# yosungho/LineTR

Measured on AMD Instinct MI355X. Metric: line_descriptors_per_sec, higher is better.
Workload: dtype f32 in/out; GEMMs as 6 bf16-split MFMA products, fp32 accumulate (fp32-faithful); 1 GPU; cfg3: 64 pairs/GPU of 640x480, 200 lines/image -> 199 sub-lines x 21 tokens, d_model=256, seeded weights; pairs_per_gpu=64, collective=none

## Files before the change

### linetr_amd/csrc/linetr_net.hip

```cpp
#include <algorithm>
#include <array>
#include <numeric>
#include <set>

#include "lt_handle.h"
#include "lt_gemm.h"
#include "lt_gemm_split.h"
#include "lt_gemm_split16.h"
#include "lt_st_image.h"
#include "lt_gemm_small.h"
#include "lt_model.h"
#include "lt_attn.h"
#include "lt_attn_fused.h"
#include "lt_gemm_ws.h"
#include "lt_tokmlp.h"
#include "lt_token.h"
#include "lt_bntrain.h"

using namespace lt;

namespace {

const char* gemm_class_name(int precision, int tile, const GemmArgs& g, int groups) {
  static const auto names = [] {
// ... 197 lines not shown
  }
  return 0;
}

int nhwc_map(LinetrHandle* h, hipStream_t st, const float* dense_desc, int dense_is_nhwc, int n_images, int P, float* buf,
             const float*& nhwc) {
  nhwc = dense_desc;
  if (dense_is_nhwc) return LINETR_OK;
  ProfScope ps(h, st, "nchw_to_nhwc", 0, 2.0 * n_images * P * D * 4);
  hipLaunchKernelGGL(nchw_to_nhwc_kernel, dim3(cdiv(P, 64), D / 64, n_images), dim3(256), 0, st, dense_desc, buf, D, P);
  LT_LAUNCH_CHECK();
  nhwc = buf;
  return LINETR_OK;
}

struct TokenFront {
  const LinetrLineRec* recs; int K, N; double td; int T;
  const float *dense_desc, *dense_score;
  int n_images, height, width, align_corners, dense_is_nhwc;
  double clip_x, clip_y;
  float *sublines, *resp, *angle_sub;
  int* s2l_g;
  float* nhwc_buf;
  bool map_always;
  double tokenize_bytes;
  float *cpnt = nullptr, *cscore = nullptr; int n_pad_images = 0; int64_t first_pad = 0;
};
int token_front(LinetrHandle* h, hipStream_t st, const TokenFront& a, const LinetrTokens& out, const K2sTable& k2s, int32_t* d_sub2line,
                const float*& nhwc) {
  {
    ProfScope ps(h, st, "line_fill", 0, (double)a.K * 80 + (double)a.N * 8);
    hipLaunchKernelGGL(line_fill_kernel, dim3(cdiv(a.K, 256)), dim3(256), 0, st, a.recs, a.K, a.clip_x, a.clip_y, out.klines, out.length,
                       out.angles, a.s2l_g, d_sub2line);
    LT_LAUNCH_CHECK();
  }
  {
    ProfScope ps(h, st, "tokenize", 0, a.tokenize_bytes);
    hipLaunchKernelGGL(tokenize_kernel, dim3(a.N + cdiv(a.n_pad_images, 64) + (out.mat ? a.K : 0)), dim3(64), 0, st, a.recs, a.s2l_g, a.N,
                       a.td, a.T, a.height, a.width, a.clip_x, a.clip_y, a.dense_score, a.sublines, out.pnt, out.mask, a.resp, a.angle_sub,
                       out.score, a.cpnt, a.cscore, a.n_pad_images, a.first_pad, out.mat, k2s);
    LT_LAUNCH_CHECK();
  }
  const int Hc = a.height / 8, Wc = a.width / 8;
  nhwc = nullptr;
  if (a.map_always || out.desc)
    if (int e = nhwc_map(h, st, a.dense_desc, a.dense_is_nhwc, a.n_images, Hc * Wc, a.nhwc_buf, nhwc)) return e;
  if (out.desc) {
    const int64_t ntok = (int64_t)a.N * a.T;
    ProfScope ps(h, st, "sample_desc", 0, (double)ntok * D * 4 * 2);
    hipLaunchKernelGGL(sample_desc_kernel, dim3((unsigned)((ntok + 3) / 4)), dim3(256), 0, st, out.pnt, a.s2l_g, a.recs, ntok, a.T, nhwc,
                       Hc, Wc, a.align_corners, out.desc);
    LT_LAUNCH_CHECK();
  }
  return LINETR_OK;
}
}

extern "C" int64_t linetr_tokenize_workspace_bytes(int32_t n_images, int32_t height, int32_t width, int32_t N) {
  const int64_t P = (int64_t)(height / 8) * (width / 8);
  return align_up(n_images * P * D * 4, 256) + align_up((int64_t)std::max(N, 1) * 4, 256) + 256;
}

extern "C" int linetr_tokenize(LinetrHandle* h, const LinetrLineRec* d_recs, int32_t K, int32_t N, double td,
                               int32_t T, const float* d_dense_desc, const float* d_dense_score, int32_t n_images,
                               int32_t height, int32_t width, int32_t clip_height, int32_t clip_width, int32_t align_corners,
// ... 8 lines not shown
  if (T < 1 || T > 4096 || height % 8 || width % 8) return fail(LINETR_E_ARG, "tokenize: bad max_tokens / image size");
  if (out.mat && n_images != 1) return fail(LINETR_E_ARG, "tokenize: mat_klines2sublines of several images: use linetr_describe (it has the sub-line prefix sums)");
  K2sTable k2s;
  if (int e = k2s_table(out, n_images, K, N, nullptr, k2s, "tokenize")) return e;
  if (ws_bytes < linetr_tokenize_workspace_bytes(n_images, height, width, N))
    return fail(LINETR_E_WORKSPACE, "tokenize: workspace too small");
  hipStream_t st = (hipStream_t)stream;
  if (h) LT_HIP(hipSetDevice(h->device));
  const int64_t P = (int64_t)(height / 8) * (width / 8);
  TokenFront f{d_recs, K, N, td, T, d_dense_desc, d_dense_score, n_images, height, width, align_corners, dense_is_nhwc,
               (double)clip_width - 0.6, (double)clip_height - 0.6, out.sublines, out.resp, out.angle_sub};
  f.nhwc_buf = (float*)d_ws;
  f.s2l_g = (int*)((char*)d_ws + align_up(n_images * P * D * 4, 256));
  f.map_always = false;
  f.tokenize_bytes = (double)N * T * 16;
  const float* nhwc;
  return token_front(h, st, f, out, k2s, d_sub2line, nhwc);
}

extern "C" int64_t linetr_sample_descriptors_workspace_bytes(int32_t Hc, int32_t Wc, int32_t dense_is_nhwc) {
  return dense_is_nhwc ? 0 : align_up((int64_t)Hc * Wc * D * 4, 256);
}

extern "C" int linetr_sample_descriptors(LinetrHandle* h, const float* d_points, int64_t n, const float* d_dense_desc, int32_t Hc,
                                         int32_t Wc, int32_t align_corners, int32_t dense_is_nhwc, float* d_out, void* d_ws,
                                         int64_t ws_bytes, void* stream) {
  if (n < 0 || Hc <= 0 || Wc <= 0) return fail(LINETR_E_ARG, "sample_descriptors: bad shape");
  if (n == 0) return LINETR_OK;
  if (!d_points || !d_dense_desc || !d_out) return fail(LINETR_E_ARG, "sample_descriptors: null pointer");
  if (ws_bytes < linetr_sample_descriptors_workspace_bytes(Hc, Wc, dense_is_nhwc) || (!dense_is_nhwc && !d_ws))
    return fail(LINETR_E_WORKSPACE, "sample_descriptors: workspace too small");
  hipStream_t st = (hipStream_t)stream;
// ... 84 lines not shown
  hipStream_t stream[LinetrHandle::PIPE_STREAMS];
  hipEvent_t ev[LinetrHandle::PIPE_STREAMS - 1];
  int cut[LinetrHandle::PIPE_STREAMS - 1];
  int n_cuts = 0, next = 0;
};
int pipe_boundary(PipeStages* p, int pos, hipStream_t& st) {
  if (!p || p->next >= p->n_cuts || p->cut[p->next] != pos) return LINETR_OK;
  LT_HIP(hipEventRecord(p->ev[p->next], st));
  LT_HIP(hipStreamWaitEvent(p->stream[p->next + 1], p->ev[p->next], 0));
  st = p->stream[++p->next];
  return LINETR_OK;
}

struct TokenStage {
  const float *pnt = nullptr, *score = nullptr, *desc = nullptr;
  const float *cpnt = nullptr, *cscore = nullptr, *nhwc = nullptr;
  const LinetrLineRec* recs = nullptr;
  const int* sub2line_g = nullptr;
  int64_t rows = 0;
  int64_t first_pad = 0;
  int Hc = 0, Wc = 0, align_corners = 0;
  const BnTrain* bn = nullptr;
  PipeStages* pipe = nullptr;
};

bool fused_mlp_enabled(const LinetrModelConfig& c) { return c.enc_channels[1] == 64 && c.enc_channels[2] == 128; }

int mlp123_rows_per_wave(int64_t rows) {
  const int64_t waves = 256 * 4;
  return (int)std::max<int64_t>(cdiv((int)cdiv((int)rows, (int)waves), 32) * 32, 32);
}
// ... 122 lines not shown
  if (ts.bn) {
    int64_t off = 0;
    if ((e = pos_encoder_bn(h, st, word, *ts.bn, off))) return e;
    if ((e = pos_encoder_bn(h, st, line, *ts.bn, off))) return e;
  } else if (plan.both >= 0) {
    ProfScope ps(h, st, "pos_mlp_dual_bf16x6", 2.0 * rows * (3 * e0 + e0 * e1 + e1 * e2 + e2 * e3) + 2.0 * N * (5 * e0 + e0 * e1 + e1 * e2 + e2 * e3),
                 (double)rows * (12 + 4 * e3) + (double)N * (28 + 4 * e3));
    if ((e = tok_mlp_launch_dual(tok_mlp_args(h, word), tok_mlp_args(h, line), st))) return e;
  } else {
    if ((e = pos_encoder(h, st, word, plan.word))) return e;
    if ((e = pos_encoder(h, st, line, plan.line))) return e;
  }
  return run_gemm(h, st, h->lW5, N, {w.act[ENC_LINE][3], e3}, {w.lpos, D}, ACT_NONE);
}

enum { POOLK_DENSE = 0, POOLK_ONLINE = 1, POOLK_ONLINE_REV = 2, POOLK_SPLIT4 = 3 };
int cls_pool_plan(bool online, int N) { return !online ? POOLK_DENSE : N <= 2048 ? POOLK_SPLIT4 : POOLK_ONLINE_REV; }

int cls_pool_launch(LinetrHandle* h, hipStream_t st, int kernel, const TokenStage& ts, int n_images, int N, int T, const float* a4,
                    float* pooled) {
  const int64_t rows = ts.rows;
  if (kernel != POOLK_DENSE) {
    const double tap_bytes = std::min((double)n_images * ts.Hc * ts.Wc * D * 4, (double)rows * D * 4 * 4);
    ProfScope ps(h, st, "cls_pool_online", 2.0 * rows * (2.0 * HEADS * D * 2), tap_bytes + (double)rows * D * 4 + (double)N * HEADS * POOLW * 4);
    if (kernel == POOLK_SPLIT4)
      hipLaunchKernelGGL(cls_pool_online_kernel<4>, dim3(N), dim3(256), 0, st, ts.recs, ts.sub2line_g, ts.cpnt,
                         a4, ts.first_pad, N, T, ts.nhwc, ts.Hc, ts.Wc, ts.align_corners, h->pool, pooled, 0);
    else
      hipLaunchKernelGGL(cls_pool_online_kernel<1>, dim3(cdiv(N, 4)), dim3(256), 0, st, ts.recs, ts.sub2line_g, ts.cpnt,
                         a4, ts.first_pad, N, T, ts.nhwc, ts.Hc, ts.Wc, ts.align_corners, h->pool, pooled, kernel == POOLK_ONLINE_REV ? 1 : 0);
    LT_LAUNCH_CHECK();
  } else {
    ProfScope ps(h, st, "cls_pool", 2.0 * rows * (2.0 * HEADS * D * 2), (double)rows * D * 8);
    hipLaunchKernelGGL(cls_pool_kernel, dim3(N), dim3(256), HEADS * (T + 1) * sizeof(float), st, ts.desc, a4, T, h->pool, pooled);
    LT_LAUNCH_CHECK();
  }
  return LINETR_OK;
}

int cls_pooling(LinetrHandle* h, hipStream_t& st, const TokenStage& ts, int n_images, int N, int T, FwdWs& w) {
  if (int e = cls_pool_launch(h, st, cls_pool_plan(ts.cpnt != nullptr, N), ts, n_images, N, T, w.act[ENC_WORD][3], w.pooled)) return e;
  const GemmGroups heads{HEADS, DH, POOLW, DH};
  return run_gemm(h, st, h->Watt, N, {w.pooled, HEADS * POOLW}, {w.att, D}, ACT_NONE, nullptr, &heads);
}

int sentence(LinetrHandle* h, hipStream_t& st, int N, FwdWs& w) {
  const LinetrModelConfig& c = h->cfg;
  int e;
  {
    NormSpec ns; ns.mode = 1; ns.gamma = h->ln1g; ns.beta = h->ln1b; ns.eps = 1e-6f;
    if ((e = run_gemm_norm(h, st, h->Wfc, N, {w.att, D}, nullptr, w.fc, w.o, ns))) return e;
  }
  if ((e = run_gemm(h, st, h->Wf1, N, {w.o, D}, {w.f1, c.d_inner}, ACT_GELU))) return e;
  NormSpec ns; ns.mode = 1; ns.gamma = h->ln2g; ns.beta = h->ln2b; ns.add2 = w.lpos; ns.eps = 1e-6f;
  return run_gemm_norm(h, st, h->Wf2, N, {w.f1, c.d_inner}, w.o, w.f2, w.zA, ns);
}
// ... 178 lines not shown
  if (!d_bn_running) return fail(LINETR_E_ARG, "forward_train: null running statistics");
  if (!(momentum >= 0.f && momentum <= 1.f)) return fail(LINETR_E_ARG, "forward_train: momentum out of [0, 1]");
  BnTrain bt;
  bt.running = d_bn_running; bt.batch = d_bn_batch; bt.momentum = momentum;
  return forward_dense(h, "forward_train", *tok, h_cu, d_cu, n_images, T, d_line_desc, d_ws, ws_bytes, (hipStream_t)stream, &bt);
}


namespace {
struct DescWs { float *nhwc, *cpnt, *cscore, *sublines, *resp, *angle_sub; int* s2l_g; int64_t fwd_off, total; };
DescWs desc_layout(int n_images, int height, int width, int N, int64_t rows, char* base) {
  DescWs d;
  int64_t off = 0;
  auto take = [&](int64_t bytes) { char* p = base + off; off += align_up(bytes, 256); return p; };
  const int64_t P = (int64_t)(height / 8) * (width / 8);
  d.nhwc = (float*)take(n_images * P * D * 4);
  d.cpnt = (float*)take(rows * 8);
  d.cscore = (float*)take(rows * 4);
  d.sublines = (float*)take((int64_t)N * 16);
  d.resp = (float*)take((int64_t)N * 4);
  d.angle_sub = (float*)take((int64_t)N * 8);
  d.s2l_g = (int*)take((int64_t)N * 4);
  d.fwd_off = off;
  d.total = off;
  return d;
}
}

extern "C" int64_t linetr_describe_workspace_bytes(const LinetrHandle* h, int32_t n_images, int32_t height, int32_t width,
                                                   int32_t N, int64_t n_real) {
  if (!h) return -1;
// ... 22 lines not shown
  if (ws_bytes < linetr_describe_workspace_bytes(h, n_images, height, width, N, n_real))
    return fail(LINETR_E_WORKSPACE, "describe: workspace too small");
  const int64_t rows = n_real + n_images;
  if (rows > INT32_MAX / 8) return fail(LINETR_E_ARG, "describe: batch too large");
  LT_HIP(hipSetDevice(h->device));
  DescWs dw = desc_layout(n_images, height, width, N, rows, (char*)d_ws);
  FwdWs w = fwd_layout(h, N, rows, n_images, (char*)d_ws + dw.fwd_off);
  const int* cu_dev;
  if (int e = cu_on_device(h_cu, d_cu, n_images, w, st, cu_dev)) return e;
  TokenFront f{d_recs, K, N, td, T, d_dense_desc, d_dense_score, n_images, height, width, align_corners, dense_is_nhwc,
               (double)width - 0.6, (double)height - 0.6, out.sublines ? out.sublines : dw.sublines, out.resp ? out.resp : dw.resp,
               out.angle_sub ? out.angle_sub : dw.angle_sub};
  f.s2l_g = dw.s2l_g; f.nhwc_buf = dw.nhwc;
  f.map_always = true;
  f.tokenize_bytes = (double)n_real * 16;
  f.cpnt = dw.cpnt; f.cscore = dw.cscore; f.n_pad_images = n_images; f.first_pad = n_real;
  const float* nhwc_map;
  if (int e = token_front(h, st, f, out, k2s, d_sub2line, nhwc_map)) return e;
  TokenStage ts;
  ts.cpnt = dw.cpnt; ts.cscore = dw.cscore; ts.nhwc = nhwc_map; ts.recs = d_recs; ts.sub2line_g = dw.s2l_g;
  ts.rows = rows; ts.first_pad = n_real; ts.Hc = height / 8; ts.Wc = width / 8; ts.align_corners = align_corners;
  ts.pipe = pipe;
  if (int e = pipe_boundary(pipe, CUT_TOKENS, st)) return e;
  return forward_core(h, st, ts, f.sublines, f.resp, f.angle_sub, h_cu, cu_dev, n_images, N, T, d_line_desc, w);
}

int pipe_ready(LinetrHandle* h) {
  LinetrHandle::Pipe& p = h->pipe;
  if (p.stream[0]) return LINETR_OK;
  if (p.failed) return fail(LINETR_E_HIP, "describe_submit: the pipeline's streams could not be created");
  constexpr int NS = LinetrHandle::PIPE_STREAMS, NL = LinetrHandle::PIPE_SLOTS, NE = NL * (NS + 1);
  hipStream_t s[NS] = {};
  hipEvent_t ev[NE] = {};
  bool ok = true;
  for (int i = 0; ok && i < NS; ++i) ok = hipStreamCreateWithFlags(&s[i], hipStreamNonBlocking) == hipSuccess;
// ... 340 lines not shown
    int64_t off = 0;
    e = pos_encoder_bn(h, st, c, bt, off);
    nb = bn_row_chunks(rows);
  }
  if (nb_used) *nb_used = nb;
  (void)hipStreamSynchronize(st);
  return e;
}

extern "C" int linetr_debug_cls_pool(LinetrHandle* h, int32_t kernel, const LinetrLineRec* d_recs, int32_t K, const int32_t* d_sub2line,
                                     int32_t N, int32_t T, const float* d_cpnt, const float* d_a4, int64_t first_pad, int32_t n_images,
                                     const float* d_map, int32_t dense_is_nhwc, int32_t Hc, int32_t Wc, int32_t align_corners,
                                     const float* d_desc_dense, float* d_pooled, int32_t* kernel_used, void* stream) {
  if (!h) return fail(LINETR_E_ARG, "debug_cls_pool: null handle");
  if (h->cfg.bn_batch_stats) return fail(LINETR_E_ARG, "debug_cls_pool: a training-mode handle (bn_batch_stats = 1) is not served");
  if (kernel < -1 || kernel > POOLK_SPLIT4) return fail(LINETR_E_ARG, "debug_cls_pool: kernel must be -1 .. 3");
  if (N < 0) return fail(LINETR_E_ARG, "debug_cls_pool: negative sub-line count");
  if (kernel == -1) kernel = cls_pool_plan(d_desc_dense == nullptr, N);
  if (kernel_used) *kernel_used = kernel;
  if (!d_pooled) return LINETR_OK;
  if (T < 1 || T > 4096) return fail(LINETR_E_ARG, "debug_cls_pool: max_tokens must be 1 .. 4096");
  if (N == 0) return LINETR_OK;
  if (!d_a4) return fail(LINETR_E_ARG, "debug_cls_pool: null tensor");
  if (((uintptr_t)d_a4 | (uintptr_t)d_pooled) % 16) return fail(LINETR_E_ARG, "debug_cls_pool: tensors must be 16-byte aligned");
  hipStream_t st = (hipStream_t)stream;
  TokenStage ts;
  if (kernel == POOLK_DENSE) {
    if (!d_desc_dense || (uintptr_t)d_desc_dense % 16) return fail(LINETR_E_ARG, "debug_cls_pool: the dense kernel reads d_desc_dense [N][T][256], 16-byte aligned");
    if ((int64_t)N * T > INT32_MAX / 8) return fail(LINETR_E_ARG, "debug_cls_pool: batch too large");
    LT_HIP(hipSetDevice(h->device));
    ts.desc = d_desc_dense; ts.rows = (int64_t)N * T;
    const int e = cls_pool_launch(h, st, kernel, ts, 1, N, T, d_a4, d_pooled);
    (void)hipStreamSynchronize(st);
    return e;
  }
  if (!d_recs || !d_sub2line || !d_cpnt || !d_map) return fail(LINETR_E_ARG, "debug_cls_pool: null tensor");
  if (K < 1 || n_images < 1 || Hc < 1 || Wc < 1 || first_pad < 0 || first_pad > INT32_MAX / 8 || (int64_t)n_images * Hc * Wc > INT32_MAX / D)
    return fail(LINETR_E_ARG, "debug_cls_pool: bad shape");
  if ((uintptr_t)d_recs % 8 || ((uintptr_t)d_sub2line | (uintptr_t)d_cpnt | (uintptr_t)d_map) % 4 || (dense_is_nhwc && (uintptr_t)d_map % 16))
    return fail(LINETR_E_ARG, "debug_cls_pool: misaligned tensor (records 8 bytes, an NHWC map 16, the others 4)");
  LT_HIP(hipSetDevice(h->device));
  {
    std::vector<LinetrLineRec> recs(K);
    std::vector<int32_t> s2l(N);
    LT_HIP(hipStreamSynchronize(st));
    LT_HIP(hipMemcpy(recs.data(), d_recs, (size_t)K * sizeof(LinetrLineRec), hipMemcpyDeviceToHost));
    LT_HIP(hipMemcpy(s2l.data(), d_sub2line, (size_t)N * sizeof(int32_t), hipMemcpyDeviceToHost));
    for (int n = 0; n < N; ++n) {
      if (s2l[n] < 0 || s2l[n] >= K) return fail(LINETR_E_ARG, "debug_cls_pool: sub-line %d maps to key-line %d, outside [0, %d)", n, s2l[n], K);
      const LinetrLineRec& r = recs[s2l[n]];
      const int64_t j = (int64_t)n - r.first_sub;
      if (j < 0 || j >= r.n_sub || j * T >= r.n_tok)
        return fail(LINETR_E_ARG, "debug_cls_pool: sub-line %d is not one of key-line %d's (first_sub %d, n_sub %d, n_tok %d)", n, s2l[n], r.first_sub, r.n_sub, r.n_tok);
      if (r.first_tok < 0 || (int64_t)r.first_tok + r.n_tok > first_pad)
        return fail(LINETR_E_ARG, "debug_cls_pool: key-line %d's tokens [%d, %d + %d) reach past first_pad = %lld", s2l[n], r.first_tok, r.first_tok, r.n_tok, (long long)first_pad);
      if (r.image < 0 || r.image >= n_images) return fail(LINETR_E_ARG, "debug_cls_pool: key-line %d's image %d outside [0, %d)", s2l[n], r.image, n_images);
    }
  }
  float* buf = nullptr;
  if (!dense_is_nhwc) LT_HIP(hipMalloc((void**)&buf, (size_t)n_images * Hc * Wc * D * sizeof(float)));
  ts.cpnt = d_cpnt; ts.recs = d_recs; ts.sub2line_g = d_sub2line; ts.rows = first_pad + n_images; ts.first_pad = first_pad;
  ts.Hc = Hc; ts.Wc = Wc; ts.align_corners = align_corners;
  int e = nhwc_map(h, st, d_map, dense_is_nhwc, n_images, Hc * Wc, buf, ts.nhwc);
  if (!e) e = cls_pool_launch(h, st, kernel, ts, n_images, N, T, d_a4, d_pooled);
  (void)hipStreamSynchronize(st);
  if (buf) (void)hipFree(buf);
  return e;
}
```

### linetr_amd/csrc/lt_common.h

```cpp
#pragma once
#include <hip/hip_runtime.h>

#include <atomic>
#include <cmath>
#include <cstdarg>
#include <cstdint>
#include <cstdio>
#include <cstring>
#include <string>
#include <vector>

#include "../../include/linetr_hip.h"

namespace lt {

constexpr int D = 256;
constexpr int HEADS = 4;
constexpr int DH = 64;
constexpr int POOLW = 544;
constexpr int WAVE = 64;

typedef float f32x4 __attribute__((ext_vector_type(4)));
typedef float f32x16 __attribute__((ext_vector_type(16)));

// ... 129 lines not shown
```

### linetr_amd/csrc/lt_model.h

```cpp
#pragma once
#include "lt_common.h"
#include "lt_token.h"
#include "lt_gemm_split.h"

namespace lt {

template <bool RELU = true>
__global__ void word_mlp1_kernel(const float* __restrict__ pnt, const float* __restrict__ score, int64_t rows,
                                 float cx, float cy, float scale, const float* __restrict__ W ,
                                 const float* __restrict__ b, float* __restrict__ out ) {
#pragma clang fp contract(off)
  const int64_t gid = (int64_t)blockIdx.x * blockDim.x + threadIdx.x;
  const int64_t row = gid >> 3;
  if (row >= rows) return;
  const int c0 = (int)(gid & 7) * 4;
  const float x = (pnt[row * 2 + 0] - cx) / scale;
  const float y = (pnt[row * 2 + 1] - cy) / scale;
  const float s = score[row];
  f32x4 o;
#pragma unroll
  for (int c = 0; c < 4; ++c) {
    const float* w = W + (c0 + c) * 3;
    float v = b[c0 + c] + w[0] * x + w[1] * y + w[2] * s;
    o[c] = RELU ? fmaxf(v, 0.f) : v;
// ... 233 lines not shown
      ab[h] += p * av;
    }
  }
  float* out = pooled + (int64_t)n * 4 * POOLW;
#pragma unroll
  for (int h = 0; h < 4; ++h) {
    out[h * POOLW + tid] = db[h];
    out[h * POOLW + 256 + tid] = ab[h];
  }
  if (tid < 4 * 32) {
    const int h = tid >> 5, i = tid & 31;
    out[h * POOLW + 512 + i] = i == 0 ? sm[h * S] : 0.f;
  }
}

template <int SPLIT>
__global__ __launch_bounds__(256, 3) void cls_pool_online_kernel(
    const LinetrLineRec* __restrict__ recs, const int* __restrict__ sub2line_g, const float* __restrict__ cpnt,
    const float* __restrict__ a4, int64_t first_pad, int N, int T, const float* __restrict__ nhwc, int Hc, int Wc,
    int align_corners, ClsPoolConst cc, float* __restrict__ pooled , int reverse) {
  const int lane = threadIdx.x & 63;
  const int wv = threadIdx.x >> 6;
  const int n_fwd = SPLIT == 1 ? blockIdx.x * 4 + wv : blockIdx.x;
  if (n_fwd >= N) return;
  const int n = reverse ? N - 1 - n_fwd : n_fwd;
  const LinetrLineRec r = recs[sub2line_g[n]];
  const int j = n - r.first_sub;
  const int n_valid = min(T, r.n_tok - j * T);
  const int n_pad = T - n_valid;
  const int ntk = n_valid + (n_pad > 0 ? 1 : 0);
  const int64_t tok0 = (int64_t)r.first_tok + (int64_t)j * T;
  const int64_t padrow = first_pad + r.image;
  const float* nhwc_img = nhwc + (int64_t)r.image * Hc * Wc * D;
  f32x4 u[4], u2[4];
#pragma unroll
// ... 6 lines not shown
#pragma unroll
  for (int h = 0; h < 4; ++h) {
    m[h] = cc.s_cls[h] * LOG2E; l[h] = 1.f; w0[h] = 1.f;
    if (SPLIT > 1 && wv != 0) { m[h] = -INFINITY; l[h] = 0.f; w0[h] = 0.f; }
    db[h] = f32x4{0.f, 0.f, 0.f, 0.f};
    ab[h] = f32x4{0.f, 0.f, 0.f, 0.f};
  }
  auto row_of = [&](int jj) -> int64_t { return jj < n_valid ? tok0 + jj : padrow; };
  int t_off[4];
  float t_w[4];
  auto fill_taps = [&](int chunk) {
    const int jj = chunk + lane;
    const int64_t row = row_of(jj < ntk ? jj : ntk - 1);
    tap_coords(cpnt[row * 2], cpnt[row * 2 + 1], Hc, Wc, align_corners, t_off, t_w);
  };
  auto issue = [&](int jj, TapSet& t, f32x4& a) {
    int off[4];
    float wt[4];
#pragma unroll
    for (int k = 0; k < 4; ++k) {
      off[k] = __builtin_amdgcn_readlane(t_off[k], jj & 63);
      wt[k] = __builtin_bit_cast(float, __builtin_amdgcn_readlane(__builtin_bit_cast(int, t_w[k]), jj & 63));
    }
    taps_load(nhwc_img, off, wt, lane, t);
    a = *reinterpret_cast<const f32x4*>(a4 + row_of(jj) * D + lane * 4);
  };
  TapSet cur, nxt;
  f32x4 a_cur, a_nxt;
  const int jj0 = SPLIT == 1 ? 0 : wv;
  fill_taps(0);
  if (jj0 < ntk) issue(jj0, cur, a_cur);
  for (int jj = jj0; jj < ntk; jj += SPLIT) {
    if (jj + SPLIT < ntk) {
      if (((jj + SPLIT) >> 6) != (jj >> 6)) fill_taps((jj + SPLIT) & ~63);
      issue(jj + SPLIT, nxt, a_nxt);
    }
    const f32x4 dv = taps_finish<true>(cur);
    const float mult = jj < n_valid ? 1.f : (float)n_pad;
    float sc[4];
#pragma unroll
    for (int h = 0; h < 4; ++h) {
      float p = 0.f;
#pragma unroll
      for (int c = 0; c < 4; ++c) p += dv[c] * u[h][c] + a_cur[c] * u2[h][c];
      sc[h] = p;
    }
    wave_sum_n<4>(sc);
#pragma unroll
    for (int h = 0; h < 4; ++h) {
      const float sh = (sc[h] + cc.c_tok[h]) * LOG2E;
      if (__any(sh > m[h])) {
        const float alpha = __builtin_amdgcn_exp2f(m[h] - sh);
        m[h] = sh;
        l[h] *= alpha;
        w0[h] *= alpha;
#pragma unroll
        for (int c = 0; c < 4; ++c) { db[h][c] *= alpha; ab[h][c] *= alpha; }
      }
      const float e = __builtin_amdgcn_exp2f(sh - m[h]) * mult;
      l[h] += e;
#pragma unroll
      for (int c = 0; c < 4; ++c) {
        db[h][c] += e * dv[c];
        ab[h][c] += e * a_cur[c];
      }
    }
    cur = nxt;
    a_cur = a_nxt;
  }
  float* out = pooled + (int64_t)n * 4 * POOLW;
  if constexpr (SPLIT > 1) {
    __shared__ float st_ml[4][4][4];
    __shared__ f32x4 st_v[4][4][2][64];
#pragma unroll
    for (int h = 0; h < 4; ++h) {
      if (lane == 0) { st_ml[wv][h][0] = m[h]; st_ml[wv][h][1] = l[h]; st_ml[wv][h][2] = w0[h]; }
      st_v[wv][h][0][lane] = db[h];
      st_v[wv][h][1][lane] = ab[h];
    }
    __syncthreads();
    const int h = wv;
    float M = st_ml[0][h][0];
#pragma unroll
// ... 76 lines not shown
```

### linetr_amd/csrc/lt_token.h

```cpp
#pragma once
#include "lt_common.h"

namespace lt {

__global__ __launch_bounds__(256) void nchw_to_nhwc_kernel(const float* __restrict__ in, float* __restrict__ out,
                                                           int C, int P) {
  __shared__ float tile[64][65];
  const int b = blockIdx.z;
  const int p0 = blockIdx.x * 64, c0 = blockIdx.y * 64;
  const float* src = in + (int64_t)b * C * P;
  float* dst = out + (int64_t)b * C * P;
  const int tid = threadIdx.x;
  {
    const int pq = (tid & 15) * 4;
#pragma unroll
    for (int i = 0; i < 4; ++i) {
      const int c = (tid >> 4) + i * 16;
      const float* row = src + (int64_t)(c0 + c) * P + p0 + pq;
      f32x4 v;
      if (p0 + pq + 3 < P && (((uintptr_t)row) & 15) == 0) v = *reinterpret_cast<const f32x4*>(row);
      else {
#pragma unroll
        for (int k = 0; k < 4; ++k) v[k] = p0 + pq + k < P ? row[k] : 0.f;
      }
// ... 177 lines not shown
  for (int k = 0; k < 4; ++k) {
    t.v[k] = *reinterpret_cast<const f32x4*>(base + (int64_t)off[k] * D);
    t.w[k] = wt[k];
  }
}

__device__ __forceinline__ void taps_issue(float px, float py, const float* __restrict__ nhwc_img, int Hc, int Wc,
                                           int align_corners, int lane, TapSet& t) {
  int off[4];
  float wt[4];
  tap_coords(px, py, Hc, Wc, align_corners, off, wt);
  taps_load(nhwc_img, off, wt, lane, t);
}

template <bool RCP = false>
__device__ __forceinline__ f32x4 taps_finish(const TapSet& t) {
#pragma clang fp contract(off)
  f32x4 o;
  float sq = 0.f;
#pragma unroll
  for (int c = 0; c < 4; ++c) {
    float v = t.v[0][c] * t.w[0];
    v = __builtin_fmaf(t.v[1][c], t.w[1], v);
    v = __builtin_fmaf(t.v[2][c], t.w[2], v);
    v = __builtin_fmaf(t.v[3][c], t.w[3], v);
    o[c] = v;
    sq += v * v;
  }
  sq = wave_sum(sq);
  const float nrm = fmaxf(sqrtf(sq), 1e-12f);
  if constexpr (RCP) {
    const float inv = 1.f / nrm;
#pragma unroll
    for (int c = 0; c < 4; ++c) o[c] = o[c] * inv;
  } else {
#pragma unroll
    for (int c = 0; c < 4; ++c) o[c] = o[c] / nrm;
  }
  return o;
}

__device__ __forceinline__ f32x4 sample_one(float px, float py, const float* __restrict__ nhwc_img, int Hc, int Wc,
                                            int align_corners, int lane) {
#pragma clang fp contract(off)
  const float s = 8.f;
  float gx = ((px - s / 2) + 0.5f) / ((float)Wc * s - s / 2 - 0.5f);
  float gy = ((py - s / 2) + 0.5f) / ((float)Hc * s - s / 2 - 0.5f);
  gx = gx * 2.f - 1.f;
  gy = gy * 2.f - 1.f;
  const float ix = grid_unnormalize(gx, Wc, align_corners), iy = grid_unnormalize(gy, Hc, align_corners);
  const float x_w = floorf(ix), y_n = floorf(iy);
  const float w = ix - x_w, e = 1.f - w, nn = iy - y_n, ss = 1.f - nn;
  const float nw = ss * e, ne = ss * w, sw = nn * e, se = nn * w;
  const int x0 = (int)x_w, y0 = (int)y_n, x1 = x0 + 1, y1 = y0 + 1;
// ... 23 lines not shown

__global__ __launch_bounds__(256) void sample_desc_kernel(
    const float* __restrict__ pnt, const int* __restrict__ sub2line_g, const LinetrLineRec* __restrict__ recs,
    int64_t n_tokens, int T, const float* __restrict__ nhwc, int Hc, int Wc, int align_corners,
    float* __restrict__ desc) {
  const int64_t tok = (int64_t)blockIdx.x * 4 + (threadIdx.x >> 6);
  if (tok >= n_tokens) return;
  const int lane = threadIdx.x & 63;
  const int n = (int)(tok / T);
  const int img = recs ? recs[sub2line_g[n]].image : 0;
  const f32x4 o = sample_one(pnt[tok * 2 + 0], pnt[tok * 2 + 1], nhwc + (int64_t)img * Hc * Wc * D, Hc, Wc,
                             align_corners, lane);
  *reinterpret_cast<f32x4*>(desc + tok * D + lane * 4) = o;
}

constexpr int KP_DESC_N = 64;
constexpr int KP_DESC_LS = KP_DESC_N + 1;
constexpr size_t KP_DESC_LDS = (size_t)D * KP_DESC_LS * 4;

__global__ __launch_bounds__(256) void sp_kp_desc_kernel(const float* __restrict__ kp, const int* __restrict__ cu_kp, int B,
                                                         const float* __restrict__ nhwc, int Hc, int Wc, int align_corners,
                                                         float* __restrict__ out) {
  extern __shared__ __attribute__((aligned(16))) float kp_tile[];
  int chunk = blockIdx.x, b = 0, start = 0, n_b = 0;
  for (; b < B; ++b) {
    start = cu_kp[b];
    n_b = cu_kp[b + 1] - start;
    const int nch = (n_b + KP_DESC_N - 1) / KP_DESC_N;
    if (chunk < nch) break;
    chunk -= nch;
// ... 19 lines not shown
```

### linetr_amd/engine_debug.py

```python
from __future__ import annotations

import ctypes as C

import numpy as np
import torch

from . import _native as nat
from ._shapes import D, ptr


class _DebugSurface:
    def debug_posenc(self, which: str, in0, in1, in2=None):
        a, b = self._f32(in0), self._f32(in1)
        c = self._f32(in2) if in2 is not None else None
        rows = int(b.shape[0])
        out = torch.empty((rows, 128), dtype=torch.float32, device=self.device)
        self._call("linetr_debug_posenc", {"word": 0, "line": 1}[which], a.data_ptr(), b.data_ptr(), ptr(c), rows, out.data_ptr())
        return out

    def debug_gemm(self, A, W, bias=None, residual=None, act=0, cache_weights=False, out=None):
        W = self._f32(W)
        if A.dtype != torch.float32 or A.device != self.device or A.stride(1) != 1:
            A = self._f32(A)
        M, K = A.shape
# ... 165 lines not shown
                rows = int(line[3])
                ins = [f32(line[0], 4 * rows, "sublines"), f32(line[1], rows, "resp"), f32(line[2], 2 * rows, "angle")]
            if out is None:
                out = torch.empty((rows, e[3]), dtype=torch.float32, device=self.device)
            res = out
        nbytes = self._L.linetr_debug_bn_train_workspace_bytes(self._h, which, rows)
        if nbytes < 0:
            raise ValueError("debug_bn_train: which must be -1, 0 or 1 and rows non-negative")
        ws = self._workspace("bn_debug", nbytes)
        used = C.c_int32(-1)
        self._call("linetr_debug_bn_train", which, pz, rows, C_, ld, f32(gamma, C_, "gamma"), f32(beta, C_, "beta"), *ins,
                   f32(out, rows * e[3], "out") if which >= 0 else None, float(momentum), f32(running, n_stats, "running"),
                   f32(batch, n_stats, "batch"), f32(affine, n_stats, "affine"), C.byref(used), ws.data_ptr(), ws.numel())
        return res, used.value

    CLS_POOL_KERNELS = ("cls_pool", "cls_pool_online", "cls_pool_online_reverse", "cls_pool_online_split4")

    def cls_pool_kernel(self, N, dense=False) -> int:
        used = C.c_int32(-1)
        self._call("linetr_debug_cls_pool", -1, None, 0, None, int(N), 1, None, None, 0, 1, None, 1, 1, 1, 0, C.c_void_p(16) if dense else None,
                   None, C.byref(used))
        return used.value

    def debug_cls_pool(self, kernel, a4, out, N, T, *, recs=None, sub2line=None, cpnt=None, first_pad=0, n_images=1, dense_map=None,
                       nhwc=True, Hc=0, Wc=0, align_corners=False, desc_dense=None):
        for t in (a4, out, cpnt, dense_map, desc_dense):
            if t is not None and (t.dtype != torch.float32 or t.device != self.device or not t.is_contiguous()):
                raise ValueError("contiguous float32 tensors on the engine's device expected")
        if out.numel() < N * 4 * 544:
            raise ValueError("out is smaller than [N, 4, 544]")
        if desc_dense is None:
            if recs.dtype != torch.uint8 or sub2line.dtype != torch.int32 or sub2line.numel() < N:
                raise ValueError("recs: uint8 bytes of LineRec[K]; sub2line: int32 [N]")
            if a4.numel() < (first_pad + n_images) * D or cpnt.numel() < (first_pad + n_images) * 2 or dense_map.numel() < n_images * Hc * Wc * D:
                raise ValueError("a4 / cpnt / dense_map are smaller than first_pad + n_images rows / n_images maps")
        elif a4.numel() < N * T * D or desc_dense.numel() < N * T * D:
# ... 52 lines not shown
```

Before: 10.59 million line-descriptors/s.

## Sample CLS-pool taps from LDS-resident NCHW planes instead of transposing to NHWC

When the dense map is NCHW, descriptors are not requested and the plane fits in LDS, a new sample_planes kernel replaces the full NCHW-to-NHWC transpose. Each block loads four channel planes of one image into LDS and bilinearly samples every token row into a channel-sliced row buffer. The online CLS pool kernel then reads one precomputed f32x4 per lane per token instead of doing four gathered taps, and the single-split variant prefetches four tokens at a time. This removes the map transpose and the scattered gather traffic, at the cost of an extra launch and a larger row workspace.

```diff
diff --git a/linetr_amd/csrc/linetr_net.hip b/linetr_amd/csrc/linetr_net.hip
--- a/linetr_amd/csrc/linetr_net.hip
+++ b/linetr_amd/csrc/linetr_net.hip
@@ -235,6 +235,28 @@
   return LINETR_OK;
 }
 
+enum { TOKSRC_MAP = 0,
+       TOKSRC_ROWS = 1 };
+int token_source_plan(const float* dense_desc, int dense_is_nhwc, bool dense_out, int n_images, int64_t P) {
+  const bool rows = !dense_is_nhwc && !dense_out && P > 0 && P % 4 == 0 && SP_CS * P * 4 <= SP_MAX_LDS && (uintptr_t)dense_desc % 16 == 0 &&
+                    n_images <= 65535;
+  return rows ? TOKSRC_ROWS : TOKSRC_MAP;
+}
+
+int sample_planes(LinetrHandle* h, hipStream_t st, const float* dense_desc, int n_images, int Hc, int Wc, int align_corners,
+                  const LinetrLineRec* recs, const int* s2l_g, const int* cu_sub, int N, const float* cpnt, int64_t first_pad, int64_t rows,
+                  float* S) {
+  LT_HIP(allow_dynamic_lds<sample_planes_kernel>(SP_MAX_LDS));
+  const int64_t P = (int64_t)Hc * Wc;
+  ProfScope ps(h, st, "sample_planes", 0, (double)n_images * P * D * 4 + (double)rows * D * 4);
+  hipLaunchKernelGGL(sample_planes_kernel, dim3(SP_SLICES, n_images), dim3(SP_THREADS), (size_t)(SP_CS * P * 4), st, dense_desc, Hc, Wc,
+                     align_corners, recs, s2l_g, cu_sub, N, cpnt, first_pad, rows, S);
+  LT_LAUNCH_CHECK();
+  return LINETR_OK;
+}
+
+struct TokenSource { const float* nhwc = nullptr; const float* srows = nullptr; };
+
 struct TokenFront {
   const LinetrLineRec* recs; int K, N; double td; int T;
   const float *dense_desc, *dense_score;
@@ -246,9 +268,10 @@
   bool map_always;
   double tokenize_bytes;
   float *cpnt = nullptr, *cscore = nullptr; int n_pad_images = 0; int64_t first_pad = 0;
+  const int* cu_sub = nullptr;
 };
 int token_front(LinetrHandle* h, hipStream_t st, const TokenFront& a, const LinetrTokens& out, const K2sTable& k2s, int32_t* d_sub2line,
-                const float*& nhwc) {
+                TokenSource& src) {
   {
     ProfScope ps(h, st, "line_fill", 0, (double)a.K * 80 + (double)a.N * 8);
     hipLaunchKernelGGL(line_fill_kernel, dim3(cdiv(a.K, 256)), dim3(256), 0, st, a.recs, a.K, a.clip_x, a.clip_y, out.klines, out.length,
@@ -263,13 +286,18 @@
     LT_LAUNCH_CHECK();
   }
   const int Hc = a.height / 8, Wc = a.width / 8;
-  nhwc = nullptr;
-  if (a.map_always || out.desc)
-    if (int e = nhwc_map(h, st, a.dense_desc, a.dense_is_nhwc, a.n_images, Hc * Wc, a.nhwc_buf, nhwc)) return e;
+  src = TokenSource{};
+  if (a.map_always && token_source_plan(a.dense_desc, a.dense_is_nhwc, out.desc != nullptr, a.n_images, (int64_t)Hc * Wc) == TOKSRC_ROWS) {
+    if (int e = sample_planes(h, st, a.dense_desc, a.n_images, Hc, Wc, a.align_corners, a.recs, a.s2l_g, a.cu_sub, a.N, a.cpnt, a.first_pad,
+                              a.first_pad + a.n_images, a.nhwc_buf)) return e;
+    src.srows = a.nhwc_buf;
+  } else if (a.map_always || out.desc) {
+    if (int e = nhwc_map(h, st, a.dense_desc, a.dense_is_nhwc, a.n_images, Hc * Wc, a.nhwc_buf, src.nhwc)) return e;
+  }
   if (out.desc) {
     const int64_t ntok = (int64_t)a.N * a.T;
     ProfScope ps(h, st, "sample_desc", 0, (double)ntok * D * 4 * 2);
-    hipLaunchKernelGGL(sample_desc_kernel, dim3((unsigned)((ntok + 3) / 4)), dim3(256), 0, st, out.pnt, a.s2l_g, a.recs, ntok, a.T, nhwc,
+    hipLaunchKernelGGL(sample_desc_kernel, dim3((unsigned)((ntok + 3) / 4)), dim3(256), 0, st, out.pnt, a.s2l_g, a.recs, ntok, a.T, src.nhwc,
                        Hc, Wc, a.align_corners, out.desc);
     LT_LAUNCH_CHECK();
   }
@@ -308,8 +336,8 @@
   f.s2l_g = (int*)((char*)d_ws + align_up(n_images * P * D * 4, 256));
   f.map_always = false;
   f.tokenize_bytes = (double)N * T * 16;
-  const float* nhwc;
-  return token_front(h, st, f, out, k2s, d_sub2line, nhwc);
+  TokenSource src;
+  return token_front(h, st, f, out, k2s, d_sub2line, src);
 }
 
 extern "C" int64_t linetr_sample_descriptors_workspace_bytes(int32_t Hc, int32_t Wc, int32_t dense_is_nhwc) {
@@ -424,7 +452,7 @@
 
 struct TokenStage {
   const float *pnt = nullptr, *score = nullptr, *desc = nullptr;
-  const float *cpnt = nullptr, *cscore = nullptr, *nhwc = nullptr;
+  const float *cpnt = nullptr, *cscore = nullptr, *nhwc = nullptr, *srows = nullptr;
   const LinetrLineRec* recs = nullptr;
   const int* sub2line_g = nullptr;
   int64_t rows = 0;
@@ -577,21 +605,27 @@
   return run_gemm(h, st, h->lW5, N, {w.act[ENC_LINE][3], e3}, {w.lpos, D}, ACT_NONE);
 }
 
-enum { POOLK_DENSE = 0, POOLK_ONLINE = 1, POOLK_ONLINE_REV = 2, POOLK_SPLIT4 = 3 };
-int cls_pool_plan(bool online, int N) { return !online ? POOLK_DENSE : N <= 2048 ? POOLK_SPLIT4 : POOLK_ONLINE_REV; }
+enum { POOLK_DENSE = 0, POOLK_ONLINE = 1, POOLK_ONLINE_REV = 2, POOLK_SPLIT4 = 3, POOLK_ROWS = 3, POOLK_LAST = POOLK_SPLIT4 + POOLK_ROWS };
+int cls_pool_plan(bool online, int N, int source = TOKSRC_MAP) {
+  return !online ? POOLK_DENSE : (N <= 2048 ? POOLK_SPLIT4 : POOLK_ONLINE_REV) + (source == TOKSRC_ROWS ? POOLK_ROWS : 0);
+}
 
 int cls_pool_launch(LinetrHandle* h, hipStream_t st, int kernel, const TokenStage& ts, int n_images, int N, int T, const float* a4,
                     float* pooled) {
   const int64_t rows = ts.rows;
   if (kernel != POOLK_DENSE) {
-    const double tap_bytes = std::min((double)n_images * ts.Hc * ts.Wc * D * 4, (double)rows * D * 4 * 4);
+    const bool srows = kernel > POOLK_SPLIT4;
+    if (srows) kernel -= POOLK_ROWS;
+    if (srows != (ts.srows != nullptr)) return fail(LINETR_E_ARG, "cls_pool: kernel and token source do not go together");
+    const double tap_bytes = srows ? (double)rows * D * 4 : std::min((double)n_images * ts.Hc * ts.Wc * D * 4, (double)rows * D * 4 * 4);
     ProfScope ps(h, st, "cls_pool_online", 2.0 * rows * (2.0 * HEADS * D * 2), tap_bytes + (double)rows * D * 4 + (double)N * HEADS * POOLW * 4);
-    if (kernel == POOLK_SPLIT4)
-      hipLaunchKernelGGL(cls_pool_online_kernel<4>, dim3(N), dim3(256), 0, st, ts.recs, ts.sub2line_g, ts.cpnt,
-                         a4, ts.first_pad, N, T, ts.nhwc, ts.Hc, ts.Wc, ts.align_corners, h->pool, pooled, 0);
-    else
-      hipLaunchKernelGGL(cls_pool_online_kernel<1>, dim3(cdiv(N, 4)), dim3(256), 0, st, ts.recs, ts.sub2line_g, ts.cpnt,
-                         a4, ts.first_pad, N, T, ts.nhwc, ts.Hc, ts.Wc, ts.align_corners, h->pool, pooled, kernel == POOLK_ONLINE_REV ? 1 : 0);
+    const int reverse = kernel == POOLK_ONLINE_REV ? 1 : 0;
+    auto launch = [&](auto kern, int blocks, const float* source) {
+      hipLaunchKernelGGL(kern, dim3(blocks), dim3(256), 0, st, ts.recs, ts.sub2line_g, ts.cpnt, a4, ts.first_pad, N, T, source, ts.Hc, ts.Wc,
+                         ts.align_corners, h->pool, pooled, reverse, rows);
+    };
+    if (kernel == POOLK_SPLIT4) srows ? launch(cls_pool_online_kernel<4, true>, N, ts.srows) : launch(cls_pool_online_kernel<4, false>, N, ts.nhwc);
+    else srows ? launch(cls_pool_online_kernel<1, true>, cdiv(N, 4), ts.srows) : launch(cls_pool_online_kernel<1, false>, cdiv(N, 4), ts.nhwc);
     LT_LAUNCH_CHECK();
   } else {
     ProfScope ps(h, st, "cls_pool", 2.0 * rows * (2.0 * HEADS * D * 2), (double)rows * D * 8);
@@ -602,7 +636,8 @@
 }
 
 int cls_pooling(LinetrHandle* h, hipStream_t& st, const TokenStage& ts, int n_images, int N, int T, FwdWs& w) {
-  if (int e = cls_pool_launch(h, st, cls_pool_plan(ts.cpnt != nullptr, N), ts, n_images, N, T, w.act[ENC_WORD][3], w.pooled)) return e;
+  const int kernel = cls_pool_plan(ts.cpnt != nullptr, N, ts.srows ? TOKSRC_ROWS : TOKSRC_MAP);
+  if (int e = cls_pool_launch(h, st, kernel, ts, n_images, N, T, w.act[ENC_WORD][3], w.pooled)) return e;
   const GemmGroups heads{HEADS, DH, POOLW, DH};
   return run_gemm(h, st, h->Watt, N, {w.pooled, HEADS * POOLW}, {w.att, D}, ACT_NONE, nullptr, &heads);
 }
@@ -811,7 +846,7 @@
   int64_t off = 0;
   auto take = [&](int64_t bytes) { char* p = base + off; off += align_up(bytes, 256); return p; };
   const int64_t P = (int64_t)(height / 8) * (width / 8);
-  d.nhwc = (float*)take(n_images * P * D * 4);
+  d.nhwc = (float*)take(std::max(n_images * P, rows) * D * 4);
   d.cpnt = (float*)take(rows * 8);
   d.cscore = (float*)take(rows * 4);
   d.sublines = (float*)take((int64_t)N * 16);
@@ -864,11 +899,11 @@
   f.s2l_g = dw.s2l_g; f.nhwc_buf = dw.nhwc;
   f.map_always = true;
   f.tokenize_bytes = (double)n_real * 16;
-  f.cpnt = dw.cpnt; f.cscore = dw.cscore; f.n_pad_images = n_images; f.first_pad = n_real;
-  const float* nhwc_map;
-  if (int e = token_front(h, st, f, out, k2s, d_sub2line, nhwc_map)) return e;
+  f.cpnt = dw.cpnt; f.cscore = dw.cscore; f.n_pad_images = n_images; f.first_pad = n_real; f.cu_sub = cu_dev;
+  TokenSource src;
+  if (int e = token_front(h, st, f, out, k2s, d_sub2line, src)) return e;
   TokenStage ts;
-  ts.cpnt = dw.cpnt; ts.cscore = dw.cscore; ts.nhwc = nhwc_map; ts.recs = d_recs; ts.sub2line_g = dw.s2l_g;
+  ts.cpnt = dw.cpnt; ts.cscore = dw.cscore; ts.nhwc = src.nhwc; ts.srows = src.srows; ts.recs = d_recs; ts.sub2line_g = dw.s2l_g;
   ts.rows = rows; ts.first_pad = n_real; ts.Hc = height / 8; ts.Wc = width / 8; ts.align_corners = align_corners;
   ts.pipe = pipe;
   if (int e = pipe_boundary(pipe, CUT_TOKENS, st)) return e;
@@ -1239,9 +1274,12 @@
                                      const float* d_desc_dense, float* d_pooled, int32_t* kernel_used, void* stream) {
   if (!h) return fail(LINETR_E_ARG, "debug_cls_pool: null handle");
   if (h->cfg.bn_batch_stats) return fail(LINETR_E_ARG, "debug_cls_pool: a training-mode handle (bn_batch_stats = 1) is not served");
-  if (kernel < -1 || kernel > POOLK_SPLIT4) return fail(LINETR_E_ARG, "debug_cls_pool: kernel must be -1 .. 3");
+  if (kernel < -1 || kernel > POOLK_LAST) return fail(LINETR_E_ARG, "debug_cls_pool: kernel must be -1 .. 6");
   if (N < 0) return fail(LINETR_E_ARG, "debug_cls_pool: negative sub-line count");
-  if (kernel == -1) kernel = cls_pool_plan(d_desc_dense == nullptr, N);
+  const int source = token_source_plan(d_map, dense_is_nhwc, false, n_images, (int64_t)Hc * Wc);
+  if (kernel > POOLK_SPLIT4 && source != TOKSRC_ROWS)
+    return fail(LINETR_E_ARG, "debug_cls_pool: kernels 4 .. 6 read rows sampled from a 16-byte aligned NCHW map of P %% 4 == 0 cells, 16 P <= %d bytes", SP_MAX_LDS);
+  if (kernel == -1) kernel = cls_pool_plan(d_desc_dense == nullptr, N, source);
   if (kernel_used) *kernel_used = kernel;
   if (!d_pooled) return LINETR_OK;
   if (T < 1 || T > 4096) return fail(LINETR_E_ARG, "debug_cls_pool: max_tokens must be 1 .. 4096");
@@ -1265,9 +1303,11 @@
   if ((uintptr_t)d_recs % 8 || ((uintptr_t)d_sub2line | (uintptr_t)d_cpnt | (uintptr_t)d_map) % 4 || (dense_is_nhwc && (uintptr_t)d_map % 16))
     return fail(LINETR_E_ARG, "debug_cls_pool: misaligned tensor (records 8 bytes, an NHWC map 16, the others 4)");
   LT_HIP(hipSetDevice(h->device));
+  std::vector<LinetrLineRec> h_recs(K);
+  std::vector<int32_t> h_s2l(N);
   {
-    std::vector<LinetrLineRec> recs(K);
-    std::vector<int32_t> s2l(N);
+    std::vector<LinetrLineRec>& recs = h_recs;
+    std::vector<int32_t>& s2l = h_s2l;
     LT_HIP(hipStreamSynchronize(st));
     LT_HIP(hipMemcpy(recs.data(), d_recs, (size_t)K * sizeof(LinetrLineRec), hipMemcpyDeviceToHost));
     LT_HIP(hipMemcpy(s2l.data(), d_sub2line, (size_t)N * sizeof(int32_t), hipMemcpyDeviceToHost));
@@ -1282,11 +1322,51 @@
       if (r.image < 0 || r.image >= n_images) return fail(LINETR_E_ARG, "debug_cls_pool: key-line %d's image %d outside [0, %d)", s2l[n], r.image, n_images);
     }
   }
+  const bool srows = kernel > POOLK_SPLIT4;
+  const int64_t rows = first_pad + n_images;
+  ts.cpnt = d_cpnt; ts.recs = d_recs; ts.sub2line_g = d_sub2line; ts.rows = rows; ts.first_pad = first_pad;
+  ts.Hc = Hc; ts.Wc = Wc; ts.align_corners = align_corners;
   float* buf = nullptr;
+  int e = LINETR_OK;
+  if (srows) {
+    std::vector<int32_t> cu(n_images + 1, 0);
+    int prev = 0;
+    for (int n = 0; n < N; ++n) {
+      const int img = h_recs[h_s2l[n]].image;
+      if (img < prev) return fail(LINETR_E_ARG, "debug_cls_pool: kernels 4 .. 6 need the sub-lines ordered by image (sub-line %d)", n);
+      for (int i = prev + 1; i <= img; ++i) cu[i] = n;
+      prev = img;
+    }
+    for (int i = prev + 1; i <= n_images; ++i) cu[i] = N;
+    auto first_tok = [&](int n) -> int64_t { return n < N ? h_recs[h_s2l[n]].first_tok : first_pad; };
+    for (int n = 0; n < N; ++n) {
+      const LinetrLineRec& r = h_recs[h_s2l[n]];
+      if (n < cu[r.image] || n >= cu[r.image + 1] || r.first_tok < first_tok(cu[r.image]) || (int64_t)r.first_tok + r.n_tok > first_tok(cu[r.image + 1]))
+        return fail(LINETR_E_ARG, "debug_cls_pool: kernels 4 .. 6 need sub-lines and tokens ordered by image (sub-line %d, image %d)", n, r.image);
+    }
+    constexpr int GUARD = 1024;
+    const size_t s_floats = (size_t)rows * D, cu_floats = (size_t)align_up(n_images + 1, 4);
+    LT_HIP(hipMalloc((void**)&buf, (s_floats + GUARD + cu_floats) * sizeof(float)));
+    const float guard = 1e4f;
+    int* d_cu = (int*)(buf + s_floats + GUARD);
+    std::vector<float> back(GUARD);
+    bool ok = hipMemsetD32Async((hipDeviceptr_t)buf, __builtin_bit_cast(int, guard), s_floats + GUARD, st) == hipSuccess &&
+              hipMemcpyAsync(d_cu, cu.data(), (size_t)(n_images + 1) * sizeof(int), hipMemcpyHostToDevice, st) == hipSuccess;
+    if (ok) {
+      e = sample_planes(h, st, d_map, n_images, Hc, Wc, align_corners, d_recs, d_sub2line, d_cu, N, d_cpnt, first_pad, rows, buf);
+      ts.srows = buf;
+      if (!e) e = cls_pool_launch(h, st, kernel, ts, n_images, N, T, d_a4, d_pooled);
+      ok = hipStreamSynchronize(st) == hipSuccess &&
+           hipMemcpy(back.data(), buf + s_floats, GUARD * sizeof(float), hipMemcpyDeviceToHost) == hipSuccess;
+    }
+    (void)hipFree(buf);
+    if (!ok) { (void)hipGetLastError(); return fail(LINETR_E_HIP, "debug_cls_pool: a HIP call around the sampled rows failed"); }
+    for (float v : back)
+      if (!e && v != guard) e = fail(LINETR_E_HIP, "debug_cls_pool: sample_planes_kernel wrote behind S");
+    return e;
+  }
   if (!dense_is_nhwc) LT_HIP(hipMalloc((void**)&buf, (size_t)n_images * Hc * Wc * D * sizeof(float)));
-  ts.cpnt = d_cpnt; ts.recs = d_recs; ts.sub2line_g = d_sub2line; ts.rows = first_pad + n_images; ts.first_pad = first_pad;
-  ts.Hc = Hc; ts.Wc = Wc; ts.align_corners = align_corners;
-  int e = nhwc_map(h, st, d_map, dense_is_nhwc, n_images, Hc * Wc, buf, ts.nhwc);
+  e = nhwc_map(h, st, d_map, dense_is_nhwc, n_images, Hc * Wc, buf, ts.nhwc);
   if (!e) e = cls_pool_launch(h, st, kernel, ts, n_images, N, T, d_a4, d_pooled);
   (void)hipStreamSynchronize(st);
   if (buf) (void)hipFree(buf);
diff --git a/linetr_amd/csrc/lt_common.h b/linetr_amd/csrc/lt_common.h
--- a/linetr_amd/csrc/lt_common.h
+++ b/linetr_amd/csrc/lt_common.h
@@ -8,6 +8,7 @@
 #include <cstdio>
 #include <cstring>
 #include <string>
+#include <type_traits>
 #include <vector>
 
 #include "../../include/linetr_hip.h"
diff --git a/linetr_amd/csrc/lt_model.h b/linetr_amd/csrc/lt_model.h
--- a/linetr_amd/csrc/lt_model.h
+++ b/linetr_amd/csrc/lt_model.h
@@ -271,11 +271,12 @@
   }
 }
 
-template <int SPLIT>
+struct RowTap { f32x4 v[1]; };
+template <int SPLIT, bool ROWS = false>
 __global__ __launch_bounds__(256, 3) void cls_pool_online_kernel(
     const LinetrLineRec* __restrict__ recs, const int* __restrict__ sub2line_g, const float* __restrict__ cpnt,
     const float* __restrict__ a4, int64_t first_pad, int N, int T, const float* __restrict__ nhwc, int Hc, int Wc,
-    int align_corners, ClsPoolConst cc, float* __restrict__ pooled , int reverse) {
+    int align_corners, ClsPoolConst cc, float* __restrict__ pooled , int reverse, int64_t rows) {
   const int lane = threadIdx.x & 63;
   const int wv = threadIdx.x >> 6;
   const int n_fwd = SPLIT == 1 ? blockIdx.x * 4 + wv : blockIdx.x;
@@ -312,59 +313,83 @@
     const int64_t row = row_of(jj < ntk ? jj : ntk - 1);
     tap_coords(cpnt[row * 2], cpnt[row * 2 + 1], Hc, Wc, align_corners, t_off, t_w);
   };
-  auto issue = [&](int jj, TapSet& t, f32x4& a) {
-    int off[4];
-    float wt[4];
-#pragma unroll
-    for (int k = 0; k < 4; ++k) {
-      off[k] = __builtin_amdgcn_readlane(t_off[k], jj & 63);
-      wt[k] = __builtin_bit_cast(float, __builtin_amdgcn_readlane(__builtin_bit_cast(int, t_w[k]), jj & 63));
-    }
-    taps_load(nhwc_img, off, wt, lane, t);
-    a = *reinterpret_cast<const f32x4*>(a4 + row_of(jj) * D + lane * 4);
+  using Tap = std::conditional_t<ROWS, RowTap, TapSet>;
+  auto issue = [&](int jj, Tap& t) {
+    if constexpr (ROWS) {
+      t.v[0] = *reinterpret_cast<const f32x4*>(nhwc + ((int64_t)lane * rows + row_of(jj)) * 4);
+    } else {
+      int off[4];
+      float wt[4];
+#pragma unroll
+      for (int k = 0; k < 4; ++k) {
+        off[k] = __builtin_amdgcn_readlane(t_off[k], jj & 63);
+        wt[k] = __builtin_bit_cast(float, __builtin_amdgcn_readlane(__builtin_bit_cast(int, t_w[k]), jj & 63));
+      }
+      taps_load(nhwc_img, off, wt, lane, t);
+    }
   };
-  TapSet cur, nxt;
+  auto a4_row = [&](int jj) { return *reinterpret_cast<const f32x4*>(a4 + row_of(jj) * D + lane * 4); };
+  constexpr int CH = (ROWS && SPLIT == 1) ? 4 : 1;
+  Tap cur[CH], nxt[CH];
   f32x4 a_cur, a_nxt;
+  auto fetch = [&](int j0, Tap (&t)[CH]) {
+#pragma unroll
+    for (int q = 0; q < CH; ++q)
+      if (j0 + q * SPLIT < ntk) issue(j0 + q * SPLIT, t[q]);
+  };
   const int jj0 = SPLIT == 1 ? 0 : wv;
-  fill_taps(0);
-  if (jj0 < ntk) issue(jj0, cur, a_cur);
-  for (int jj = jj0; jj < ntk; jj += SPLIT) {
-    if (jj + SPLIT < ntk) {
-      if (((jj + SPLIT) >> 6) != (jj >> 6)) fill_taps((jj + SPLIT) & ~63);
-      issue(jj + SPLIT, nxt, a_nxt);
-    }
-    const f32x4 dv = taps_finish<true>(cur);
-    const float mult = jj < n_valid ? 1.f : (float)n_pad;
-    float sc[4];
-#pragma unroll
-    for (int h = 0; h < 4; ++h) {
-      float p = 0.f;
-#pragma unroll
-      for (int c = 0; c < 4; ++c) p += dv[c] * u[h][c] + a_cur[c] * u2[h][c];
-      sc[h] = p;
-    }
-    wave_sum_n<4>(sc);
-#pragma unroll
-    for (int h = 0; h < 4; ++h) {
-      const float sh = (sc[h] + cc.c_tok[h]) * LOG2E;
-      if (__any(sh > m[h])) {
-        const float alpha = __builtin_amdgcn_exp2f(m[h] - sh);
-        m[h] = sh;
-        l[h] *= alpha;
-        w0[h] *= alpha;
-#pragma unroll
-        for (int c = 0; c < 4; ++c) { db[h][c] *= alpha; ab[h][c] *= alpha; }
-      }
-      const float e = __builtin_amdgcn_exp2f(sh - m[h]) * mult;
-      l[h] += e;
-#pragma unroll
-      for (int c = 0; c < 4; ++c) {
-        db[h][c] += e * dv[c];
-        ab[h][c] += e * a_cur[c];
-      }
-    }
-    cur = nxt;
-    a_cur = a_nxt;
+  if constexpr (!ROWS) fill_taps(0);
+  if (jj0 < ntk) {
+    fetch(jj0, cur);
+    a_cur = a4_row(jj0);
+  }
+  for (int j0 = jj0; j0 < ntk; j0 += SPLIT * CH) {
+    if (j0 + SPLIT * CH < ntk) {
+      if constexpr (!ROWS)
+        if (((j0 + SPLIT) >> 6) != (j0 >> 6)) fill_taps((j0 + SPLIT) & ~63);
+      fetch(j0 + SPLIT * CH, nxt);
+    }
+#pragma unroll
+    for (int q = 0; q < CH; ++q) {
+      const int jj = j0 + q * SPLIT;
+      if (jj >= ntk) break;
+      if (jj + SPLIT < ntk) a_nxt = a4_row(jj + SPLIT);
+      f32x4 dv;
+      if constexpr (ROWS) dv = unit_norm<true>(cur[q].v[0]);
+      else dv = taps_finish<true>(cur[q]);
+      const float mult = jj < n_valid ? 1.f : (float)n_pad;
+      float sc[4];
+#pragma unroll
+      for (int h = 0; h < 4; ++h) {
+        float p = 0.f;
+#pragma unroll
+        for (int c = 0; c < 4; ++c) p += dv[c] * u[h][c] + a_cur[c] * u2[h][c];
+        sc[h] = p;
+      }
+      wave_sum_n<4>(sc);
+#pragma unroll
+      for (int h = 0; h < 4; ++h) {
+        const float sh = (sc[h] + cc.c_tok[h]) * LOG2E;
+        if (__any(sh > m[h])) {
+          const float alpha = __builtin_amdgcn_exp2f(m[h] - sh);
+          m[h] = sh;
+          l[h] *= alpha;
+          w0[h] *= alpha;
+#pragma unroll
+          for (int c = 0; c < 4; ++c) { db[h][c] *= alpha; ab[h][c] *= alpha; }
+        }
+        const float e = __builtin_amdgcn_exp2f(sh - m[h]) * mult;
+        l[h] += e;
+#pragma unroll
+        for (int c = 0; c < 4; ++c) {
+          db[h][c] += e * dv[c];
+          ab[h][c] += e * a_cur[c];
+        }
+      }
+      a_cur = a_nxt;
+    }
+#pragma unroll
+    for (int q = 0; q < CH; ++q) cur[q] = nxt[q];
   }
   float* out = pooled + (int64_t)n * 4 * POOLW;
   if constexpr (SPLIT > 1) {
diff --git a/linetr_amd/csrc/lt_token.h b/linetr_amd/csrc/lt_token.h
--- a/linetr_amd/csrc/lt_token.h
+++ b/linetr_amd/csrc/lt_token.h
@@ -215,19 +215,11 @@
 }
 
 template <bool RCP = false>
-__device__ __forceinline__ f32x4 taps_finish(const TapSet& t) {
-#pragma clang fp contract(off)
-  f32x4 o;
+__device__ __forceinline__ f32x4 unit_norm(f32x4 o) {
+#pragma clang fp contract(off)
   float sq = 0.f;
 #pragma unroll
-  for (int c = 0; c < 4; ++c) {
-    float v = t.v[0][c] * t.w[0];
-    v = __builtin_fmaf(t.v[1][c], t.w[1], v);
-    v = __builtin_fmaf(t.v[2][c], t.w[2], v);
-    v = __builtin_fmaf(t.v[3][c], t.w[3], v);
-    o[c] = v;
-    sq += v * v;
-  }
+  for (int c = 0; c < 4; ++c) sq += o[c] * o[c];
   sq = wave_sum(sq);
   const float nrm = fmaxf(sqrtf(sq), 1e-12f);
   if constexpr (RCP) {
@@ -239,6 +231,23 @@
     for (int c = 0; c < 4; ++c) o[c] = o[c] / nrm;
   }
   return o;
+}
+
+__device__ __forceinline__ float taps_blend(float nw, float ne, float sw, float se, const float (&w)[4]) {
+#pragma clang fp contract(off)
+  float v = nw * w[0];
+  v = __builtin_fmaf(ne, w[1], v);
+  v = __builtin_fmaf(sw, w[2], v);
+  v = __builtin_fmaf(se, w[3], v);
+  return v;
+}
+
+template <bool RCP = false>
+__device__ __forceinline__ f32x4 taps_finish(const TapSet& t) {
+  f32x4 o;
+#pragma unroll
+  for (int c = 0; c < 4; ++c) o[c] = taps_blend(t.v[0][c], t.v[1][c], t.v[2][c], t.v[3][c], t.w);
+  return unit_norm<RCP>(o);
 }
 
 __device__ __forceinline__ f32x4 sample_one(float px, float py, const float* __restrict__ nhwc_img, int Hc, int Wc,
@@ -292,6 +301,57 @@
   *reinterpret_cast<f32x4*>(desc + tok * D + lane * 4) = o;
 }
 
+constexpr int SP_CS = 4;
+constexpr int SP_SLICES = D / SP_CS;
+constexpr int SP_THREADS = 1024;
+constexpr int SP_MAX_LDS = 80 * 1024;
+constexpr int SP_PIECES = SP_MAX_LDS / 16 / SP_THREADS;
+
+__global__ __launch_bounds__(SP_THREADS, 8) void sample_planes_kernel(
+    const float* __restrict__ nchw, int Hc, int Wc, int align_corners, const LinetrLineRec* __restrict__ recs,
+    const int* __restrict__ sub2line_g, const int* __restrict__ cu_sub, int N, const float* __restrict__ cpnt, int64_t first_pad,
+    int64_t rows, float* __restrict__ S) {
+  extern __shared__ __attribute__((aligned(16))) float sp_planes[];
+  const int slice = blockIdx.x, img = blockIdx.y;
+  const int P = Hc * Wc;
+  const f32x4* src = reinterpret_cast<const f32x4*>(nchw + ((int64_t)img * D + slice * SP_CS) * P);
+  f32x4 piece[SP_PIECES];
+#pragma unroll
+  for (int k = 0; k < SP_PIECES; ++k) {
+    const int i = threadIdx.x + k * SP_THREADS;
+    if (i < P) piece[k] = src[i];
+  }
+  const int n0 = cu_sub[img], n1 = cu_sub[img + 1];
+  const int64_t t0 = max((int64_t)0, n0 < N ? (int64_t)recs[sub2line_g[n0]].first_tok : first_pad);
+  const int64_t t1 = min(first_pad, n1 < N ? (int64_t)recs[sub2line_g[n1]].first_tok : first_pad);
+  int off[4];
+  float wt[4];
+  int64_t t = t0 + threadIdx.x, row = 0;
+  auto geometry = [&] {
+    row = t < t1 ? t : first_pad + img;
+    tap_coords(cpnt[row * 2], cpnt[row * 2 + 1], Hc, Wc, align_corners, off, wt);
+  };
+  if (t <= t1) geometry();
+#pragma unroll
+  for (int k = 0; k < SP_PIECES; ++k) {
+    const int i = threadIdx.x + k * SP_THREADS;
+    if (i < P) reinterpret_cast<f32x4*>(sp_planes)[i] = piece[k];
+  }
+  __syncthreads();
+  float* out = S + (int64_t)slice * rows * SP_CS;
+  while (t <= t1) {
+    f32x4 o;
+#pragma unroll
+    for (int c = 0; c < SP_CS; ++c) {
+      const float* pl = sp_planes + c * P;
+      o[c] = taps_blend(pl[off[0]], pl[off[1]], pl[off[2]], pl[off[3]], wt);
+    }
+    *reinterpret_cast<f32x4*>(out + row * SP_CS) = o;
+    t += SP_THREADS;
+    if (t <= t1) geometry();
+  }
+}
+
 constexpr int KP_DESC_N = 64;
 constexpr int KP_DESC_LS = KP_DESC_N + 1;
 constexpr size_t KP_DESC_LDS = (size_t)D * KP_DESC_LS * 4;
diff --git a/linetr_amd/engine_debug.py b/linetr_amd/engine_debug.py
--- a/linetr_amd/engine_debug.py
+++ b/linetr_amd/engine_debug.py
@@ -203,12 +203,14 @@
                    f32(batch, n_stats, "batch"), f32(affine, n_stats, "affine"), C.byref(used), ws.data_ptr(), ws.numel())
         return res, used.value
 
-    CLS_POOL_KERNELS = ("cls_pool", "cls_pool_online", "cls_pool_online_reverse", "cls_pool_online_split4")
-
-    def cls_pool_kernel(self, N, dense=False) -> int:
-        used = C.c_int32(-1)
-        self._call("linetr_debug_cls_pool", -1, None, 0, None, int(N), 1, None, None, 0, 1, None, 1, 1, 1, 0, C.c_void_p(16) if dense else None,
-                   None, C.byref(used))
+    CLS_POOL_KERNELS = ("cls_pool", "cls_pool_online", "cls_pool_online_reverse", "cls_pool_online_split4",
+                        "sample_planes + cls_pool_online<rows>", "sample_planes + cls_pool_online_reverse<rows>",
+                        "sample_planes + cls_pool_online_split4<rows>")
+
+    def cls_pool_kernel(self, N, dense=False, nhwc=True, hw_cells=(1, 1), n_images=1, map_ptr=0) -> int:
+        used = C.c_int32(-1)
+        self._call("linetr_debug_cls_pool", -1, None, 0, None, int(N), 1, None, None, 0, int(n_images), C.c_void_p(int(map_ptr)) if map_ptr else None,
+                   int(bool(nhwc)), int(hw_cells[0]), int(hw_cells[1]), 0, C.c_void_p(16) if dense else None, None, C.byref(used))
         return used.value
 
     def debug_cls_pool(self, kernel, a4, out, N, T, *, recs=None, sub2line=None, cpnt=None, first_pad=0, n_images=1, dense_map=None,
```

Result: no change. 10.68 million line-descriptors/s, median of 6 (+0.8%).
